# dfm/george

Hardware: NVIDIA H100
Metric: gp.compute+log_likelihood N-points/sec (higher is better)
Workload: dtype f64

## Files before the change

george_b200/csrc/hodlr_leaf.cuh:

```cuda
#pragma once

#include "gemm_dmma.cuh"
#include "hodlr_kernels.cuh"

namespace bgp {

constexpr int LF_THREADS = 256;
constexpr int LF_NB = 32;
constexpr int LF_MAX_LEAF = 768;
constexpr int LF_LDW = 40;

__host__ __device__ inline int lf_panel_ld(int max_m) { return ((max_m + 15) / 16) * 16 + 8; }

__device__ __forceinline__ void lf_axpy(double* dst, int ds, const double* src, int ss, int lo, int hi, double f) {
  for (int j0 = lo; j0 <= hi; j0 += 8) {
    double a[8], b[8];
#pragma unroll
    for (int u = 0; u < 8; ++u)
      if (j0 + u <= hi) { a[u] = dst[(j0 + u) * ds]; b[u] = src[(j0 + u) * ss]; }
#pragma unroll
    for (int u = 0; u < 8; ++u)
      if (j0 + u <= hi) dst[(j0 + u) * ds] = a[u] - f * b[u];
  }
}

template <int SHAPE>
__global__ void __launch_bounds__(LF_THREADS, 2) leaf_factor_kernel(const DevProgram* __restrict__ gprog,
                                                                    const double* __restrict__ x,
                                                                    const double* __restrict__ diag,
                                                                    const LeafDesc* __restrict__ leaves,
                                                                    double* __restrict__ Lbuf,
                                                                    double* __restrict__ leaf_logdet, int ldp) {
  extern __shared__ __align__(16) double lf_smem[];
  double* pn = lf_smem;
  double* dall = lf_smem + LF_NB * ldp;
  double* w11 = dall + ldp;
  DevProgram* P = reinterpret_cast<DevProgram*>(w11 + LF_NB * LF_LDW);
  __shared__ double red[32];
  if constexpr (SHAPE == BGP_SHAPE_GENERIC) stage_program(P, gprog);
  __syncthreads();
  const auto fn = ShapeEval<SHAPE>::make(P, gprog);
  const LeafDesc lf = leaves[blockIdx.x];
  const int m = lf.size, nd = gprog->ndim;
  double* A = Lbuf + lf.off;
  const double* xs = x + (int64_t)lf.start * nd;
  const int lane = threadIdx.x & 31, warp = threadIdx.x >> 5;
  const int lr = lane >> 2, lc = lane & 3;

  constexpr int LF_BUILD_ILP = SHAPE == BGP_SHAPE_GENERIC ? 1 : 4;
  double logdet = 0.0;
  for (int k0 = 0; k0 < m; k0 += LF_NB) {
    const int nb = min(LF_NB, m - k0), rem = m - k0;
    for (int t0 = threadIdx.x; t0 < nb * rem; t0 += LF_BUILD_ILP * LF_THREADS) {
      double v[LF_BUILD_ILP];
#pragma unroll
      for (int u = 0; u < LF_BUILD_ILP; ++u) {
        const int t = t0 + u * LF_THREADS, c = t / rem, i = t - c * rem;
        v[u] = (t < nb * rem && i >= c) ? fn(xs + (int64_t)(k0 + i) * nd, xs + (int64_t)(k0 + c) * nd) : 0.0;
      }
#pragma unroll
      for (int u = 0; u < LF_BUILD_ILP; ++u) {
        const int t = t0 + u * LF_THREADS, c = t / rem, i = t - c * rem;
        if (t < nb * rem && i >= c) pn[c * ldp + i] = (i == c) ? v[u] + diag[lf.start + k0 + i] : v[u];
      }
    }
    __syncthreads();
    if (k0 > 0) {
      const int n_tiles = (rem + 15) / 16;
      bool bok[4];
#pragma unroll
      for (int b = 0; b < 4; ++b) bok[b] = b * 8 + lr < nb;
      for (int t = warp; t < n_tiles; t += LF_THREADS / 32) {
        const int r0 = t * 16;
        bool aok[2];
#pragma unroll
        for (int a = 0; a < 2; ++a) aok[a] = r0 + a * 8 + lr < rem;
        double acc[2][4][2];
#pragma unroll
        for (int a = 0; a < 2; ++a)
#pragma unroll
          for (int b = 0; b < 4; ++b) { acc[a][b][0] = 0.0; acc[a][b][1] = 0.0; }
#pragma unroll 4
        for (int q0 = 0; q0 < k0; q0 += 4) {
          const int q = q0 + lc;
          const double* Lq = A + (int64_t)q * m + k0;
          const double dq = dall[q];
          double af[2], bf[4];
#pragma unroll
          for (int a = 0; a < 2; ++a) af[a] = aok[a] ? Lq[r0 + a * 8 + lr] : 0.0;
#pragma unroll
          for (int b = 0; b < 4; ++b) bf[b] = bok[b] ? Lq[b * 8 + lr] * dq : 0.0;
#pragma unroll
          for (int a = 0; a < 2; ++a)
#pragma unroll
            for (int b = 0; b < 4; ++b) dmma884(acc[a][b][0], acc[a][b][1], af[a], bf[b]);
        }
#pragma unroll
        for (int a = 0; a < 2; ++a) {
          const int i = r0 + a * 8 + lr;
#pragma unroll
          for (int b = 0; b < 4; ++b)
#pragma unroll
            for (int e = 0; e < 2; ++e) {
              const int c = b * 8 + 2 * lc + e;
              if (i < rem && c < nb && i >= c) pn[c * ldp + i] -= acc[a][b][e];
            }
        }
      }
      __syncthreads();
    }
    if (warp == 0) {
      double* t11 = w11;
      for (int j = 0; j < LF_NB; ++j) t11[j * LF_LDW + lane] = (j == lane) ? 1.0 : 0.0;
      __syncwarp();
      for (int k = 0; k < nb; ++k) {
        const double d = pn[k * ldp + k];
        const bool below = lane > k && lane < nb;
        const double l = below ? pn[k * ldp + lane] / d : 0.0;
        if (below) pn[k * ldp + lane] = l;
        __syncwarp();
        if (below) {
          const double ld = l * d;
          lf_axpy(pn + lane, ldp, pn + k * ldp, 1, k + 1, lane, ld);
          lf_axpy(t11 + lane, LF_LDW, t11 + k, LF_LDW, 0, k, l);
        }
        __syncwarp();
      }
      if (lane < nb) {
        const double d = pn[lane * ldp + lane];
        const double dinv = 1.0 / d;
        double* col = A + (int64_t)k0 * m + k0 + lane;
        for (int j = 0; j < lane; ++j) col[(int64_t)j * m] = pn[j * ldp + lane];
        col[(int64_t)lane * m] = d;
        dall[k0 + lane] = d;
        logdet += log(fabs(d));
        for (int j = 0; j <= lane; ++j) t11[j * LF_LDW + lane] *= dinv;
      }
    }
    __syncthreads();
    if (rem > LF_NB) {
      const int n_tiles = (rem - LF_NB + 15) / 16;
      for (int t = warp; t < n_tiles; t += LF_THREADS / 32) {
        const int r0 = LF_NB + t * 16;
        bool aok[2];
#pragma unroll
        for (int a = 0; a < 2; ++a) aok[a] = r0 + a * 8 + lr < rem;
        double acc[2][4][2];
#pragma unroll
        for (int a = 0; a < 2; ++a)
#pragma unroll
          for (int b = 0; b < 4; ++b) { acc[a][b][0] = 0.0; acc[a][b][1] = 0.0; }
#pragma unroll
        for (int q0 = 0; q0 < LF_NB; q0 += 4) {
          const int q = q0 + lc;
          double af[2], bf[4];
#pragma unroll
          for (int a = 0; a < 2; ++a) af[a] = aok[a] ? pn[q * ldp + r0 + a * 8 + lr] : 0.0;
#pragma unroll
          for (int b = 0; b < 4; ++b) bf[b] = w11[q * LF_LDW + b * 8 + lr];
#pragma unroll
          for (int a = 0; a < 2; ++a)
#pragma unroll
            for (int b = 0; b < 4; ++b) dmma884(acc[a][b][0], acc[a][b][1], af[a], bf[b]);
        }
#pragma unroll
        for (int a = 0; a < 2; ++a) {
          const int i = r0 + a * 8 + lr;
          if (i < rem) {
#pragma unroll
            for (int b = 0; b < 4; ++b)
#pragma unroll
              for (int e = 0; e < 2; ++e) A[(int64_t)(k0 + b * 8 + 2 * lc + e) * m + k0 + i] = acc[a][b][e];
          }
        }
      }
    }
    __syncthreads();
  }
  logdet = block_sum(logdet, red);
  if (threadIdx.x == 0) leaf_logdet[blockIdx.x] = logdet;
}

__host__ inline size_t lf_smem_bytes(int shape, int max_m) {
  return sizeof(double) * ((size_t)(LF_NB + 1) * lf_panel_ld(max_m) + LF_NB * LF_LDW) +
         (shape == BGP_SHAPE_GENERIC ? sizeof(DevProgram) : 0);
}

template <int SHAPE>
inline void leaf_factor_launch_shape(int n_leaves, int max_m, cudaStream_t s, const DevProgram* prog, const double* x,
                                     const double* diag, const LeafDesc* leaves, double* L, double* leaf_logdet) {
  const size_t smem = lf_smem_bytes(SHAPE, max_m);
  cudaFuncSetAttribute(leaf_factor_kernel<SHAPE>, cudaFuncAttributeMaxDynamicSharedMemorySize, (int)smem);
  leaf_factor_kernel<SHAPE><<<n_leaves, LF_THREADS, smem, s>>>(prog, x, diag, leaves, L, leaf_logdet, lf_panel_ld(max_m));
}

inline void leaf_factor_launch(int shape, int n_leaves, int max_m, cudaStream_t s, const DevProgram* prog,
                               const double* x, const double* diag, const LeafDesc* leaves, double* L,
                               double* leaf_logdet) {
  BGP_SHAPE_SWITCH(shape, (leaf_factor_launch_shape<SHAPE>(n_leaves, max_m, s, prog, x, diag, leaves, L, leaf_logdet)));
}

}
```

Before: 24.62 million.

## Overlap next panel build and Schur update with warp-0 diagonal factorization

While warp 0 factors the current 32-wide diagonal block, the other seven warps now build the next panel's kernel values straight into global L and precompute most of its trailing update. That partial update is parked in unused upper-triangle storage of A. The main update then only adds the last panel's contribution, so warps that used to sit idle during the serial factorization do useful work. The cost is more complex indexing, extra global traffic for the parked accumulators, and reliance on that scratch region being free.

```diff
diff --git a/george_b200/csrc/hodlr_leaf.cuh b/george_b200/csrc/hodlr_leaf.cuh
--- a/george_b200/csrc/hodlr_leaf.cuh
+++ b/george_b200/csrc/hodlr_leaf.cuh
@@ -37,6 +37,7 @@
   double* w11 = dall + ldp;
   DevProgram* P = reinterpret_cast<DevProgram*>(w11 + LF_NB * LF_LDW);
   __shared__ double red[32];
+  __shared__ double draw[LF_NB];
   if constexpr (SHAPE == BGP_SHAPE_GENERIC) stage_program(P, gprog);
   __syncthreads();
   const auto fn = ShapeEval<SHAPE>::make(P, gprog);
@@ -48,67 +49,86 @@
   const int lr = lane >> 2, lc = lane & 3;
 
   constexpr int LF_BUILD_ILP = SHAPE == BGP_SHAPE_GENERIC ? 1 : 4;
+  auto build = [&](int kp, int t_first, int nthreads) {
+    const int nb = min(LF_NB, m - kp), rem = m - kp;
+    for (int t0 = t_first; t0 < nb * rem; t0 += LF_BUILD_ILP * nthreads) {
+      double v[LF_BUILD_ILP];
+#pragma unroll
+      for (int u = 0; u < LF_BUILD_ILP; ++u) {
+        const int t = t0 + u * nthreads, c = t / rem, i = t - c * rem;
+        v[u] = (t < nb * rem && i >= c) ? fn(xs + (int64_t)(kp + i) * nd, xs + (int64_t)(kp + c) * nd) : 0.0;
+      }
+#pragma unroll
+      for (int u = 0; u < LF_BUILD_ILP; ++u) {
+        const int t = t0 + u * nthreads, c = t / rem, i = t - c * rem;
+        if (t < nb * rem && i > c) A[(int64_t)(kp + c) * m + kp + i] = v[u];
+        if (t < nb * rem && i == c) draw[c] = v[u] + diag[lf.start + kp + i];
+      }
+    }
+  };
+  auto update = [&](double (&acc)[2][4][2], int kp, int r0, int q_lo, int q_hi) {
+    const int nb = min(LF_NB, m - kp), rem = m - kp;
+    bool aok[2], bok[4];
+#pragma unroll
+    for (int a = 0; a < 2; ++a) aok[a] = r0 + a * 8 + lr < rem;
+#pragma unroll
+    for (int b = 0; b < 4; ++b) bok[b] = b * 8 + lr < nb;
+#pragma unroll 4
+    for (int q0 = q_lo; q0 < q_hi; q0 += 4) {
+      const int q = q0 + lc;
+      const double* Lq = A + (int64_t)q * m + kp;
+      const double dq = dall[q];
+      double af[2], bf[4];
+#pragma unroll
+      for (int a = 0; a < 2; ++a) af[a] = aok[a] ? Lq[r0 + a * 8 + lr] : 0.0;
+#pragma unroll
+      for (int b = 0; b < 4; ++b) bf[b] = bok[b] ? Lq[b * 8 + lr] * dq : 0.0;
+#pragma unroll
+      for (int a = 0; a < 2; ++a)
+#pragma unroll
+        for (int b = 0; b < 4; ++b) dmma884(acc[a][b][0], acc[a][b][1], af[a], bf[b]);
+    }
+  };
+  auto parked = [&](int t, int a, int b, int e) -> double& {
+    return A[(int64_t)(LF_NB + 16 * t + 8 * a + 2 * b + e) * m + lane];
+  };
+
   double logdet = 0.0;
+  build(0, threadIdx.x, LF_THREADS);
+  __syncthreads();
   for (int k0 = 0; k0 < m; k0 += LF_NB) {
-    const int nb = min(LF_NB, m - k0), rem = m - k0;
-    for (int t0 = threadIdx.x; t0 < nb * rem; t0 += LF_BUILD_ILP * LF_THREADS) {
-      double v[LF_BUILD_ILP];
-#pragma unroll
-      for (int u = 0; u < LF_BUILD_ILP; ++u) {
-        const int t = t0 + u * LF_THREADS, c = t / rem, i = t - c * rem;
-        v[u] = (t < nb * rem && i >= c) ? fn(xs + (int64_t)(k0 + i) * nd, xs + (int64_t)(k0 + c) * nd) : 0.0;
-      }
-#pragma unroll
-      for (int u = 0; u < LF_BUILD_ILP; ++u) {
-        const int t = t0 + u * LF_THREADS, c = t / rem, i = t - c * rem;
-        if (t < nb * rem && i >= c) pn[c * ldp + i] = (i == c) ? v[u] + diag[lf.start + k0 + i] : v[u];
-      }
+    const int nb = min(LF_NB, m - k0), rem = m - k0, k1 = k0 + LF_NB;
+    for (int t = warp; t < (rem + 15) / 16; t += LF_THREADS / 32) {
+      const int r0 = t * 16;
+      double acc[2][4][2];
+#pragma unroll
+      for (int a = 0; a < 2; ++a)
+#pragma unroll
+        for (int b = 0; b < 4; ++b)
+#pragma unroll
+          for (int e = 0; e < 2; ++e) acc[a][b][e] = k0 > LF_NB ? parked(t, a, b, e) : 0.0;
+      update(acc, k0, r0, max(k0 - LF_NB, 0), k0);
+#pragma unroll
+      for (int a = 0; a < 2; ++a)
+#pragma unroll
+        for (int b = 0; b < 4; ++b)
+#pragma unroll
+          for (int e = 0; e < 2; ++e) {
+            const int i = r0 + a * 8 + lr, c = b * 8 + 2 * lc + e;
+            if (i < rem && c < nb && i >= c)
+              acc[a][b][e] = (i == c ? draw[c] : A[(int64_t)(k0 + c) * m + k0 + i]) - acc[a][b][e];
+          }
+#pragma unroll
+      for (int a = 0; a < 2; ++a)
+#pragma unroll
+        for (int b = 0; b < 4; ++b)
+#pragma unroll
+          for (int e = 0; e < 2; ++e) {
+            const int i = r0 + a * 8 + lr, c = b * 8 + 2 * lc + e;
+            if (i < rem && c < nb && i >= c) pn[c * ldp + i] = acc[a][b][e];
+          }
     }
     __syncthreads();
-    if (k0 > 0) {
-      const int n_tiles = (rem + 15) / 16;
-      bool bok[4];
-#pragma unroll
-      for (int b = 0; b < 4; ++b) bok[b] = b * 8 + lr < nb;
-      for (int t = warp; t < n_tiles; t += LF_THREADS / 32) {
-        const int r0 = t * 16;
-        bool aok[2];
-#pragma unroll
-        for (int a = 0; a < 2; ++a) aok[a] = r0 + a * 8 + lr < rem;
-        double acc[2][4][2];
-#pragma unroll
-        for (int a = 0; a < 2; ++a)
-#pragma unroll
-          for (int b = 0; b < 4; ++b) { acc[a][b][0] = 0.0; acc[a][b][1] = 0.0; }
-#pragma unroll 4
-        for (int q0 = 0; q0 < k0; q0 += 4) {
-          const int q = q0 + lc;
-          const double* Lq = A + (int64_t)q * m + k0;
-          const double dq = dall[q];
-          double af[2], bf[4];
-#pragma unroll
-          for (int a = 0; a < 2; ++a) af[a] = aok[a] ? Lq[r0 + a * 8 + lr] : 0.0;
-#pragma unroll
-          for (int b = 0; b < 4; ++b) bf[b] = bok[b] ? Lq[b * 8 + lr] * dq : 0.0;
-#pragma unroll
-          for (int a = 0; a < 2; ++a)
-#pragma unroll
-            for (int b = 0; b < 4; ++b) dmma884(acc[a][b][0], acc[a][b][1], af[a], bf[b]);
-        }
-#pragma unroll
-        for (int a = 0; a < 2; ++a) {
-          const int i = r0 + a * 8 + lr;
-#pragma unroll
-          for (int b = 0; b < 4; ++b)
-#pragma unroll
-            for (int e = 0; e < 2; ++e) {
-              const int c = b * 8 + 2 * lc + e;
-              if (i < rem && c < nb && i >= c) pn[c * ldp + i] -= acc[a][b][e];
-            }
-        }
-      }
-      __syncthreads();
-    }
     if (warp == 0) {
       double* t11 = w11;
       for (int j = 0; j < LF_NB; ++j) t11[j * LF_LDW + lane] = (j == lane) ? 1.0 : 0.0;
@@ -136,6 +156,25 @@
         logdet += log(fabs(d));
         for (int j = 0; j <= lane; ++j) t11[j * LF_LDW + lane] *= dinv;
       }
+    } else if (k1 < m) {
+      build(k1, threadIdx.x - 32, LF_THREADS - 32);
+      if (k0 > 0) {
+        for (int t = warp - 1; t < (m - k1 + 15) / 16; t += LF_THREADS / 32 - 1) {
+          const int r0 = t * 16;
+          double acc[2][4][2];
+#pragma unroll
+          for (int a = 0; a < 2; ++a)
+#pragma unroll
+            for (int b = 0; b < 4; ++b) { acc[a][b][0] = 0.0; acc[a][b][1] = 0.0; }
+          update(acc, k1, r0, 0, k0);
+#pragma unroll
+          for (int a = 0; a < 2; ++a)
+#pragma unroll
+            for (int b = 0; b < 4; ++b)
+#pragma unroll
+              for (int e = 0; e < 2; ++e) parked(t, a, b, e) = acc[a][b][e];
+        }
+      }
     }
     __syncthreads();
     if (rem > LF_NB) {
```

Result: faster. 25.43 million, median of 6 (+3.3%).
